# facebookresearch/actionmesh

Measured on AMD Instinct MI355X. Metric: denoise-steps/sec (16f x 4096tok), higher is better.
Workload: dtype bf16; 1 GPU; headline: Stage-I denoise step, B=2 (CFG) x T=16 frames x N=4096 tokens, width 1024 (8 heads x 128), 21 layers all inflated, S=257 ctx tokens, random-init weights, seeded N(0,1) latents/context resident in HBM; parallelism=single GPU

## Files before the change

actionmesh_amd/csrc/am_gemm.hip:

```cpp
#include <stdlib.h>
#include <string.h>

#include "am_common.h"

namespace {

constexpr int BM = 128, BN = 128, BK = 64;
constexpr int LDS_ROW = BK + 8;
constexpr int TILE_ELEMS = BM * LDS_ROW;
constexpr int CS_LD = BN + 4;
constexpr int SMEM_MAIN = 2 * 2 * TILE_ELEMS * (int)sizeof(bf16_t);
constexpr int SMEM_EPI = BM * CS_LD * (int)sizeof(float);
constexpr int SMEM_BYTES = SMEM_MAIN > SMEM_EPI ? SMEM_MAIN : SMEM_EPI;
constexpr int GROUP_M = 8;
constexpr int B2 = 256;

__device__ inline int64_t map_row(int r, int G, int gs, int off) {
  if (G <= 0) return r;
  int g = r / G;
  return (int64_t)g * gs + off + (r - g * G);
}

__global__ __launch_bounds__(256, 2) void gemm_bf16_kernel(am_gemm_args p, int tiles_m, int tiles_n, int m_base) {
  extern __shared__ __attribute__((aligned(16))) unsigned char smem[];
  bf16_t* As = reinterpret_cast<bf16_t*>(smem);
  bf16_t* Bs = As + 2 * TILE_ELEMS;
  float* Cs = reinterpret_cast<float*>(smem);

  const int nb = tiles_m * tiles_n;
  const int bid = blockIdx.x;
  int lid;
  {
    const int xcd = bid & 7, idx = bid >> 3;
    const int q = nb >> 3, r = nb & 7;
    lid = (xcd < r ? xcd * (q + 1) : r * (q + 1) + (xcd - r) * q) + idx;
  }
  int tm, tn;
  {
    const int group_sz = GROUP_M * tiles_n;
    const int g = lid / group_sz;
    const int first_m = g * GROUP_M;
    const int gm = min(GROUP_M, tiles_m - first_m);
    const int in_g = lid - g * group_sz;
    tm = first_m + in_g % gm;
    tn = in_g / gm;
  }
  const int m0 = m_base + tm * BM, n0 = tn * BN;

  const int tid = threadIdx.x;
  const int lane = tid & 63, wave = tid >> 6;
  const int l31 = lane & 31, hi = lane >> 5;
  const int wm = wave >> 1, wn = wave & 1;

  const bf16_t* a1p[4];
  const bf16_t* a2p[4];
  const bf16_t* wp[4];
  int lds_off[4];
#pragma unroll
  for (int i = 0; i < 4; ++i) {
    const int c = tid + 256 * i;
    const int row = c >> 3, col = (c & 7) * 8;
    const int ar = min(m0 + row, p.M - 1);
    const int64_t pr = map_row(ar, p.a_G, p.a_gs, p.a_off);
    a1p[i] = p.A1 + pr * p.lda1 + col;
    a2p[i] = p.A2 ? p.A2 + pr * p.lda2 + col - p.K1 : nullptr;
    const int wr = min(n0 + row, p.N - 1);
    wp[i] = p.W + (int64_t)wr * p.ldw + col;
    lds_off[i] = row * LDS_ROW + col;
  }

  f32x16_t acc[2][2];
#pragma unroll
  for (int i = 0; i < 2; ++i)
#pragma unroll
    for (int j = 0; j < 2; ++j)
#pragma unroll
      for (int r = 0; r < 16; ++r) acc[i][j][r] = 0.f;

  u32x4_t areg[4], wreg[4];
  auto load_tile = [&](int kt) {
    const int k0 = kt * BK;
    const bool first = k0 < p.K1;
#pragma unroll
    for (int i = 0; i < 4; ++i) {
      const bf16_t* src = first ? a1p[i] + k0 : a2p[i] + k0;
      areg[i] = *reinterpret_cast<const u32x4_t*>(src);
      wreg[i] = *reinterpret_cast<const u32x4_t*>(wp[i] + k0);
    }
  };
  auto store_tile = [&](int buf) {
#pragma unroll
    for (int i = 0; i < 4; ++i) {
      *reinterpret_cast<u32x4_t*>(&As[buf * TILE_ELEMS + lds_off[i]]) = areg[i];
      *reinterpret_cast<u32x4_t*>(&Bs[buf * TILE_ELEMS + lds_off[i]]) = wreg[i];
    }
  };

  const int nk = p.K / BK;
  load_tile(0);
  store_tile(0);

  const int a_frag_off = (wm * 64 + l31) * LDS_ROW + hi * 8;
  const int b_frag_off = (wn * 64 + l31) * LDS_ROW + hi * 8;

  for (int kt = 0; kt < nk; ++kt) {
    __syncthreads();
    const int buf = kt & 1;
    if (kt + 1 < nk) load_tile(kt + 1);
    const bf16_t* Ab = As + buf * TILE_ELEMS + a_frag_off;
    const bf16_t* Bb = Bs + buf * TILE_ELEMS + b_frag_off;
#pragma unroll
    for (int ks = 0; ks < BK / 16; ++ks) {
      bf16x8_t af[2], bfr[2];
#pragma unroll
      for (int i = 0; i < 2; ++i) {
        af[i] = *reinterpret_cast<const bf16x8_t*>(Ab + i * 32 * LDS_ROW + ks * 16);
        bfr[i] = *reinterpret_cast<const bf16x8_t*>(Bb + i * 32 * LDS_ROW + ks * 16);
      }
#pragma unroll
      for (int i = 0; i < 2; ++i)
#pragma unroll
        for (int j = 0; j < 2; ++j)
          acc[i][j] = AM_MFMA_32x32x16(bfr[j], af[i], acc[i][j]);
    }
    if (kt + 1 < nk) store_tile(buf ^ 1);
  }

  __syncthreads();
#pragma unroll
  for (int i = 0; i < 2; ++i)
#pragma unroll
    for (int j = 0; j < 2; ++j)
#pragma unroll
      for (int g = 0; g < 4; ++g) {
        const int m = wm * 64 + i * 32 + l31;
        const int n = wn * 64 + j * 32 + 8 * g + 4 * hi;
        f32x4_t v = {acc[i][j][4 * g], acc[i][j][4 * g + 1], acc[i][j][4 * g + 2], acc[i][j][4 * g + 3]};
        *reinterpret_cast<f32x4_t*>(&Cs[m * CS_LD + n]) = v;
      }
  __syncthreads();

  const int c8 = (tid & 15) * 8;
  const int gn = n0 + c8;
  if (gn < p.N) {
    float bv[8], cs[8];
#pragma unroll
    for (int e = 0; e < 8; ++e) {
      bv[e] = p.bias ? p.bias[gn + e] : 0.f;
      cs[e] = p.ln_stats ? p.ln_colsum[gn + e] : 0.f;
    }
#pragma unroll
    for (int pass = 0; pass < BM / 16; ++pass) {
      const int row = pass * 16 + (tid >> 4);
      const int gmr = m0 + row;
      if (gmr < p.M) {
        const int64_t pr = map_row(gmr, p.c_G, p.c_gs, p.c_off);
        const f32x4_t v0 = *reinterpret_cast<const f32x4_t*>(&Cs[row * CS_LD + c8]);
        const f32x4_t v1 = *reinterpret_cast<const f32x4_t*>(&Cs[row * CS_LD + c8 + 4]);
        float v[8] = {v0[0], v0[1], v0[2], v0[3], v1[0], v1[1], v1[2], v1[3]};
        if (p.ln_stats) {
          const f32x2_t st = *reinterpret_cast<const f32x2_t*>(p.ln_stats + 2 * map_row(gmr, p.a_G, p.a_gs, p.a_off));
          const float nm = -st[0] * st[1];
#pragma unroll
          for (int e = 0; e < 8; ++e) v[e] = rbf(fmaf(v[e], st[1], fmaf(nm, cs[e], bv[e])));
        } else {
#pragma unroll
          for (int e = 0; e < 8; ++e) v[e] = rbf(v[e] + bv[e]);
        }
        if ((p.act & AM_GEMM_ACT_MASK) == AM_GEMM_ACT_GELU) {
#pragma unroll
          for (int e = 0; e < 8; ++e) v[e] = rbf(gelu_erf(v[e]));
        }
        if (p.residual) {
          const u32x4_t rv = *reinterpret_cast<const u32x4_t*>(p.residual + pr * p.ldc + gn);
#pragma unroll
          for (int e = 0; e < 4; ++e) {
            v[2 * e] += bflo(rv[e]);
            v[2 * e + 1] += bfhi(rv[e]);
          }
        }
        u32x4_t o;
#pragma unroll
        for (int e = 0; e < 4; ++e) o[e] = pack_bf2(v[2 * e], v[2 * e + 1]);
        *reinterpret_cast<u32x4_t*>(p.C + pr * p.ldc + gn) = o;
      }
    }
  }
}


constexpr int TAIL_LD = 64 + 4;
__global__ __launch_bounds__(512) void gemm_tail_kernel(am_gemm_args p, int m_base) {
  __shared__ float red[4][32][TAIL_LD];
  const int tid = threadIdx.x;
  const int lane = tid & 63, wave = tid >> 6;
  const int l31 = lane & 31, hi = lane >> 5;
  const int wn = wave & 1, wk = wave >> 1;
  const int m0 = m_base + blockIdx.y * 32, nb0 = blockIdx.x * 64;
  const int ar = min(m0 + l31, p.M - 1);
  const int wr = min(nb0 + wn * 32 + l31, p.N - 1);
  const bf16_t* a1 = p.A1 + (int64_t)ar * p.lda1 + hi * 8;
  const bf16_t* a2 = p.A2 ? p.A2 + (int64_t)ar * p.lda2 + hi * 8 - p.K1 : nullptr;
  const bf16_t* wp = p.W + (int64_t)wr * p.ldw + hi * 8;
  const int kq = p.K >> 2;
  const int k_begin = wk * kq, k_end = k_begin + kq;
  f32x16_t acc;
#pragma unroll
  for (int r = 0; r < 16; ++r) acc[r] = 0.f;
  for (int k0 = k_begin; k0 < k_end; k0 += 128) {
    u32x4_t af[8], wf[8];
#pragma unroll
    for (int s = 0; s < 8; ++s) {
      const int k = min(k0 + s * 16, k_end - 16);
      af[s] = *reinterpret_cast<const u32x4_t*>((k < p.K1 ? a1 : a2) + k);
      wf[s] = *reinterpret_cast<const u32x4_t*>(wp + k);
    }
#pragma unroll
    for (int s = 0; s < 8; ++s)
      if (k0 + s * 16 < k_end)
        acc = AM_MFMA_32x32x16(__builtin_bit_cast(bf16x8_t, wf[s]), __builtin_bit_cast(bf16x8_t, af[s]), acc);
  }
#pragma unroll
  for (int g = 0; g < 4; ++g)
    *reinterpret_cast<f32x4_t*>(&red[wk][l31][wn * 32 + 8 * g + 4 * hi]) = f32x4_t{acc[4 * g], acc[4 * g + 1], acc[4 * g + 2], acc[4 * g + 3]};
  __syncthreads();
  const int row = tid >> 4, c4 = (tid & 15) * 4;
  const int gmr = m0 + row, gn = nb0 + c4;
  if (gmr >= p.M || gn >= p.N) return;
  float v[4];
  {
    const f32x4_t s0 = *reinterpret_cast<const f32x4_t*>(&red[0][row][c4]), s1 = *reinterpret_cast<const f32x4_t*>(&red[1][row][c4]);
    const f32x4_t s2 = *reinterpret_cast<const f32x4_t*>(&red[2][row][c4]), s3 = *reinterpret_cast<const f32x4_t*>(&red[3][row][c4]);
#pragma unroll
    for (int e = 0; e < 4; ++e) v[e] = (s0[e] + s1[e]) + (s2[e] + s3[e]);
  }
  float bv[4] = {0.f, 0.f, 0.f, 0.f};
  if (p.bias) {
    const f32x4_t b = *reinterpret_cast<const f32x4_t*>(p.bias + gn);
#pragma unroll
    for (int e = 0; e < 4; ++e) bv[e] = b[e];
  }
  if (p.ln_stats) {
    const f32x2_t st = *reinterpret_cast<const f32x2_t*>(p.ln_stats + 2 * (int64_t)gmr);
    const f32x4_t cs = *reinterpret_cast<const f32x4_t*>(p.ln_colsum + gn);
    const float nm = -st[0] * st[1];
#pragma unroll
    for (int e = 0; e < 4; ++e) v[e] = rbf(fmaf(v[e], st[1], fmaf(nm, cs[e], bv[e])));
  } else {
#pragma unroll
    for (int e = 0; e < 4; ++e) v[e] = rbf(v[e] + bv[e]);
  }
  if ((p.act & AM_GEMM_ACT_MASK) == AM_GEMM_ACT_GELU) {
#pragma unroll
    for (int e = 0; e < 4; ++e) v[e] = rbf(gelu_erf(v[e]));
  }
  if (p.residual) {
    const u32x2_t rv = *reinterpret_cast<const u32x2_t*>(p.residual + (int64_t)gmr * p.ldc + gn);
    v[0] += bflo(rv[0]); v[1] += bfhi(rv[0]); v[2] += bflo(rv[1]); v[3] += bfhi(rv[1]);
  }
  *reinterpret_cast<u32x2_t*>(p.C + (int64_t)gmr * p.ldc + gn) = u32x2_t{pack_bf2(v[0], v[1]), pack_bf2(v[2], v[3])};
}

#ifndef AM_GEMM_NT
#define AM_GEMM_NT 1
#endif
struct ResidualPrefetch {
  u32x4_t rv[16];
  bool on;
};
__device__ __forceinline__ bool residual_prefetchable(const am_gemm_args& p, int tid, int m0, int n0) {
  return p.residual != nullptr && p.c_G <= 0 && m0 + B2 <= p.M && n0 + (tid & 31) * 8 < p.N && !(p.act & AM_GEMM_ABLATE_MASK);
}
__device__ __forceinline__ void residual_prefetch(const am_gemm_args& p, int tid, int m0, int n0, ResidualPrefetch& r) {
  r.on = residual_prefetchable(p, tid, m0, n0);
  if (r.on) {
    const int k16 = tid & 31, r16 = tid >> 5;
    const uint32_t lane_off = ((uint32_t)r16 * (uint32_t)p.ldc + (uint32_t)(n0 + k16 * 8)) * 2u;
    const int64_t step = (int64_t)16 * p.ldc;
    const bf16_t* rrow = p.residual + (int64_t)m0 * p.ldc;
#pragma unroll
    for (int pass = 0; pass < 16; ++pass) {
      const u32x4_t* q = reinterpret_cast<const u32x4_t*>(reinterpret_cast<const unsigned char*>(rrow + pass * step) + lane_off);
      r.rv[pass] = AM_GEMM_NT ? __builtin_nontemporal_load(q) : *q;
    }
  }
}

__device__ __forceinline__ void emit_row_part(const u32x4_t& sv, float* part_row, bool writer) {
  float x[8];
#pragma unroll
  for (int e = 0; e < 4; ++e) { x[2 * e] = bflo(sv[e]); x[2 * e + 1] = bfhi(sv[e]); }
  float mean, m2;
  row_part8(x, mean, m2);
#define AM_CHAN_STEP(CTRL, ROWMASK, HALF_N)                                                                                  \
  {                                                                                                                          \
    const float om = __builtin_bit_cast(float, __builtin_amdgcn_update_dpp(__builtin_bit_cast(int, mean), __builtin_bit_cast(int, mean), CTRL, ROWMASK, 0xf, false)); \
    const float oq = __builtin_bit_cast(float, __builtin_amdgcn_update_dpp(__builtin_bit_cast(int, m2), __builtin_bit_cast(int, m2), CTRL, ROWMASK, 0xf, false));     \
    row_part_merge_equal(mean, m2, om, oq, HALF_N);                                                                          \
  }
  AM_CHAN_STEP(0xB1, 0xf, 4.f)
  AM_CHAN_STEP(0x4E, 0xf, 8.f)
  AM_CHAN_STEP(0x141, 0xf, 16.f)
  AM_CHAN_STEP(0x140, 0xf, 32.f)
  AM_CHAN_STEP(0x142, 0xa, 64.f)
#undef AM_CHAN_STEP
  if (writer) *reinterpret_cast<f32x2_t*>(part_row) = f32x2_t{mean, m2};
// ... 112 lines not shown
        u32x4_t u = *reinterpret_cast<const u32x4_t*>(su + pass * 8192);
        if (odd) u = u32x4_t{u[2], u[3], u[0], u[1]};
        float v[8];
#pragma unroll
        for (int e = 0; e < 4; ++e) {
          v[2 * e] = bflo(u[e]);
          v[2 * e + 1] = bfhi(u[e]);
        }
        if (wt) {
          float ss = 0.f;
#pragma unroll
          for (int e = 0; e < 8; ++e) ss = __builtin_fmaf(v[e], v[e], ss);
          ss += __builtin_bit_cast(float, __builtin_amdgcn_update_dpp(0, __builtin_bit_cast(int, ss), 0x128, 0xf, 0xf, false));
          ss += __builtin_bit_cast(float, __builtin_amdgcn_update_dpp(0, __builtin_bit_cast(int, ss), 0x124, 0xf, 0xf, false));
          ss += __builtin_bit_cast(float, __builtin_amdgcn_update_dpp(0, __builtin_bit_cast(int, ss), 0x122, 0xf, 0xf, false));
          ss += __builtin_bit_cast(float, __builtin_amdgcn_update_dpp(0, __builtin_bit_cast(int, ss), 0x121, 0xf, 0xf, false));
          const float r = rsqrtf(ss * (1.0f / 128.0f) + hp.eps);
#pragma unroll
          for (int e = 0; e < 8; ++e) v[e] = (v[e] * r) * wv[e];
        }
        if (hp.rope_cos) {
          f32x4_t cs, sn;
          if (two) {
            const bool nx = gm >= fb;
#pragma unroll
            for (int e = 0; e < 4; ++e) { cs[e] = nx ? cs1[e] : cs0[e]; sn[e] = nx ? sn1[e] : sn0[e]; }
          } else {
            const int frame = gm / hp.rows_per_frame;
            cs = *reinterpret_cast<const f32x4_t*>(hp.rope_cos + (int64_t)frame * 64 + sub * 4);
            sn = *reinterpret_cast<const f32x4_t*>(hp.rope_sin + (int64_t)frame * 64 + sub * 4);
          }
#pragma unroll
          for (int e = 0; e < 4; ++e) rope_rotate(v[2 * e], v[2 * e + 1], cs[e], sn[e]);
        }
        u32x4_t w;
#pragma unroll
        for (int e = 0; e < 4; ++e) w[e] = pack_bf2(v[2 * e], v[2 * e + 1]);
        if (two) {
          *reinterpret_cast<u32x4_t*>((gm >= sb ? out1 : out0) + (int64_t)gm * 128) = w;
        } else {
          const int seq = gm / hp.seq_len, sq = gm - seq * hp.seq_len;
          *reinterpret_cast<u32x4_t*>(out + (((int64_t)seq * hp.heads + head) * s_pad + sq) * 128 + sub * 8) = w;
        }
      };
      if (two && m0 + B2 <= p.M && wt != nullptr) {
        const bool rope = hp.rope_cos != nullptr;
#pragma unroll 1
        for (int b4 = 0; b4 < 16; b4 += 4) {
          u32x4_t u[4];
#pragma unroll
          for (int i = 0; i < 4; ++i) u[i] = *reinterpret_cast<const u32x4_t*>(su + (b4 + i) * 8192);
          float v[4][8], ss[4];
#pragma unroll
          for (int i = 0; i < 4; ++i) {
            if (odd) u[i] = u32x4_t{u[i][2], u[i][3], u[i][0], u[i][1]};
#pragma unroll
            for (int e = 0; e < 4; ++e) { v[i][2 * e] = bflo(u[i][e]); v[i][2 * e + 1] = bfhi(u[i][e]); }
            ss[i] = 0.f;
#pragma unroll
            for (int e = 0; e < 8; ++e) ss[i] = __builtin_fmaf(v[i][e], v[i][e], ss[i]);
          }
#define AM_HP_DPP(CTRL)                                                                                                         \
          _Pragma("unroll") for (int i = 0; i < 4; ++i)                                                                         \
            ss[i] += __builtin_bit_cast(float, __builtin_amdgcn_update_dpp(0, __builtin_bit_cast(int, ss[i]), CTRL, 0xf, 0xf, false));
          AM_HP_DPP(0x128) AM_HP_DPP(0x124) AM_HP_DPP(0x122) AM_HP_DPP(0x121)
#undef AM_HP_DPP
#pragma unroll
          for (int i = 0; i < 4; ++i) {
            const int gm = m0 + (b4 + i) * 16 + r16;
            const float r = __builtin_amdgcn_rsqf(ss[i] * (1.0f / 128.0f) + hp.eps);
#pragma unroll
            for (int e = 0; e < 8; ++e) v[i][e] = (v[i][e] * r) * wv[e];
            if (rope) {
              const bool nx = gm >= fb;
#pragma unroll
              for (int e = 0; e < 4; ++e) rope_rotate(v[i][2 * e], v[i][2 * e + 1], nx ? cs1[e] : cs0[e], nx ? sn1[e] : sn0[e]);
            }
            u32x4_t w;
#pragma unroll
            for (int e = 0; e < 4; ++e) w[e] = pack_bf2(v[i][2 * e], v[i][2 * e + 1]);
            *reinterpret_cast<u32x4_t*>((gm >= sb ? out1 : out0) + (int64_t)gm * 128) = w;
          }
        }
      } else if (two) {
#pragma unroll 4
        for (int pass = 0; pass < 16; ++pass) one_row(pass);
      } else {
#pragma unroll 2
        for (int pass = 0; pass < 16; ++pass) one_row(pass);
      }
    }
  }
  if (abl_nov) return;
#pragma unroll
  for (int h2 = 0; h2 < 2; ++h2) {
    const int pi = (n0 >> 7) + h2;
    const int head = pi / hp.nparts, part = pi - head * hp.nparts;
    if (n0 + h2 * 128 >= p.N || hp.kinds[part] != 2) continue;
    const int lane = tid & 63, wave = tid >> 6;
#pragma unroll 2
    for (int it = 0; it < 8; ++it) {
      const int pc = (lane & 7) + 8 * (it & 3);
      const int d = ((lane >> 3) & 7) + 8 * (wave + 8 * (it >> 2));
      const int pos0 = pc * 8;
      const int g16 = m0 + (pos0 & ~15);
      if (g16 >= p.M) continue;
      const int n = h2 * 128 + d;
      uint32_t val[8];
#pragma unroll
      for (int j = 0; j < 8; ++j) {
        const int pos = pos0 + j;
        const int m = (pos & ~15) | perm16(pos & 15);
        val[j] = *reinterpret_cast<const uint16_t*>(stage + m * 512 + ((((n >> 2) ^ (m & 15))) << 3) + (n & 3) * 2);
      }
      const u32x4_t w = {val[0] | (val[1] << 16), val[2] | (val[3] << 16), val[4] | (val[5] << 16), val[6] | (val[7] << 16)};
      const int seq = g16 / hp.seq_len, s16 = g16 - seq * hp.seq_len;
      *reinterpret_cast<u32x4_t*>(hp.out_vt + (((int64_t)seq * hp.heads + head) * 128 + d) * hp.sk_pad + s16 + (pos0 & 15)) = w;
    }
  }
}

constexpr int T2_UNITS = B2 * (BK / 8);
constexpr int T2_BYTES = T2_UNITS * 16;
constexpr int SMEM2_BYTES = 4 * T2_BYTES;

typedef __attribute__((address_space(3))) void* lds_ptr_t;
typedef const __attribute__((address_space(1))) void* gbl_ptr_t;

__global__ __launch_bounds__(512, 2) void gemm256_bf16_kernel(am_gemm_args p, int tiles_m, int tiles_n, int m_base) {
  extern __shared__ __attribute__((aligned(16))) unsigned char smem[];

  const int nb = tiles_m * tiles_n;
  const int bid = blockIdx.x;
  int lid;
  {
    const int xcd = bid & 7, idx = bid >> 3;
    const int q = nb >> 3, r = nb & 7;
    lid = (xcd < r ? xcd * (q + 1) : r * (q + 1) + (xcd - r) * q) + idx;
  }
  int tm, tn;
  {
    const int group_sz = GROUP_M * tiles_n;
    const int g = lid / group_sz;
    const int first_m = g * GROUP_M;
    const int gm = min(GROUP_M, tiles_m - first_m);
    const int in_g = lid - g * group_sz;
    tm = first_m + in_g % gm;
    tn = in_g / gm;
  }
  const int m0 = m_base + tm * B2, n0 = tn * B2;

  const int tid = threadIdx.x;
  const int lane = tid & 63;
  const int wave = __builtin_amdgcn_readfirstlane(tid >> 6);
  const int l31 = lane & 31, hi = lane >> 5;
  const int wm = wave >> 2, wn = wave & 3;

  const bf16_t* a1p[4];
  const bf16_t* a2p[4];
  const bf16_t* wp[4];
#pragma unroll
  for (int j = 0; j < 4; ++j) {
    const int U = j * 512 + wave * 64 + lane;
    const int r = U >> 3, c = (U & 7) ^ ((r >> 1) & 7);
    const int ar = min(m0 + r, p.M - 1);
    const int64_t pr = map_row(ar, p.a_G, p.a_gs, p.a_off);
    a1p[j] = p.A1 + pr * p.lda1 + c * 8;
    a2p[j] = p.A2 ? p.A2 + pr * p.lda2 + c * 8 - p.K1 : nullptr;
    const int wr = min(n0 + r, p.N - 1);
    wp[j] = p.W + (int64_t)wr * p.ldw + c * 8;
  }
  auto dma_pair = [&](int kt, int buf, int j) __attribute__((always_inline)) {
    const int k0 = kt * BK;
    unsigned char* abase = smem + buf * 2 * T2_BYTES;
    unsigned char* bbase = abase + T2_BYTES;
    const bf16_t* src = k0 < p.K1 ? a1p[j] + k0 : a2p[j] + k0;
    __builtin_amdgcn_global_load_lds((gbl_ptr_t)src, (lds_ptr_t)(abase + (j * 512 + wave * 64) * 16), 16, 0, 0);
    __builtin_amdgcn_global_load_lds((gbl_ptr_t)(wp[j] + k0), (lds_ptr_t)(bbase + (j * 512 + wave * 64) * 16), 16, 0, 0);
  };
  auto dma_tile = [&](int kt, int buf) {
#pragma unroll
    for (int j = 0; j < 4; ++j) dma_pair(kt, buf, j);
  };

  f32x16_t acc[4][2];
#pragma unroll
  for (int j = 0; j < 2; ++j)
#pragma unroll
    for (int g = 0; g < 4; ++g) {
      f32x4_t bv = {0.f, 0.f, 0.f, 0.f};
      if (p.bias) bv = *reinterpret_cast<const f32x4_t*>(p.bias + min(n0 + wn * 64 + j * 32 + 8 * g + 4 * hi, p.N - 4));
#pragma unroll
      for (int i = 0; i < 4; ++i)
#pragma unroll
        for (int e = 0; e < 4; ++e) acc[i][j][4 * g + e] = bv[e];
    }

  int a_row_off[4], a_sw[4], b_row_off[2], b_sw[2];
#pragma unroll
  for (int i = 0; i < 4; ++i) {
    const int R = wm * 128 + i * 32 + l31;
    a_row_off[i] = R * 128;
    a_sw[i] = (R >> 1) & 7;
  }
#pragma unroll
  for (int j = 0; j < 2; ++j) {
    const int R = wn * 64 + j * 32 + l31;
    b_row_off[j] = R * 128;
    b_sw[j] = (R >> 1) & 7;
  }

  const int nk = p.K / BK;
  dma_tile(0, 0);
  dma_drain_barrier();
  for (int kt = 0; kt < nk; ++kt) {
    const int buf = kt & 1;
    const int kn = min(kt + 1, nk - 1);
    const unsigned char* At = smem + buf * 2 * T2_BYTES;
    const unsigned char* Bt = At + T2_BYTES;
#pragma unroll
    for (int ks = 0; ks < BK / 16; ++ks) {
      if (ks < 2) {
        dma_pair(kn, buf ^ 1, 2 * ks);
        dma_pair(kn, buf ^ 1, 2 * ks + 1);
      }
      __builtin_amdgcn_sched_barrier(0);
      const int c = ks * 2 + hi;
      bf16x8_t af[4], bfr[2];
#pragma unroll
      for (int j = 0; j < 2; ++j)
        bfr[j] = *reinterpret_cast<const bf16x8_t*>(Bt + b_row_off[j] + ((c ^ b_sw[j]) << 4));
#pragma unroll
      for (int i = 0; i < 4; ++i)
        af[i] = *reinterpret_cast<const bf16x8_t*>(At + a_row_off[i] + ((c ^ a_sw[i]) << 4));
#pragma unroll
      for (int i = 0; i < 4; ++i)
#pragma unroll
        for (int j = 0; j < 2; ++j)
          acc[i][j] = AM_MFMA_32x32x16(bfr[j], af[i], acc[i][j]);
    }
    dma_drain_barrier();
  }

  unsigned char* stage = smem;
#pragma unroll
  for (int j = 0; j < 2; ++j)
#pragma unroll
    for (int g = 0; g < 4; ++g) {
      const int nl = wn * 64 + j * 32 + 8 * g + 4 * hi;
#pragma unroll
      for (int i = 0; i < 4; ++i) {
        const int ml = wm * 128 + i * 32 + l31;
        u32x2_t w;
        if ((p.act & AM_GEMM_ACT_MASK) == AM_GEMM_ACT_GELU) {
          float v[4];
#pragma unroll
          for (int e = 0; e < 4; ++e) v[e] = gelu_erf(rbf(acc[i][j][4 * g + e]));
          w = u32x2_t{pack_bf2(v[0], v[1]), pack_bf2(v[2], v[3])};
        } else {
          w = u32x2_t{pack_bf2(acc[i][j][4 * g], acc[i][j][4 * g + 1]), pack_bf2(acc[i][j][4 * g + 2], acc[i][j][4 * g + 3])};
        }
        const int u = (nl >> 2) ^ (ml & 15);
        *reinterpret_cast<u32x2_t*>(stage + ml * 512 + u * 8) = w;
      }
    }
  __syncthreads();
  store_staged_tile(p, stage, tid, m0, n0);
}


constexpr uint32_t GT_LO = (127u - 17u) << 7, GT_HI = (127u + 3u) << 7, GT_SPAN = GT_HI - GT_LO;
constexpr int GT_ENTRIES = 2 * (int)GT_SPAN;
constexpr int GT_BYTES = GT_ENTRIES * 2;
__global__ void gelu_table_kernel(uint16_t* tab) {
  const int i = blockIdx.x * blockDim.x + threadIdx.x;
  if (i >= GT_ENTRIES) return;
  const uint32_t sgn = (uint32_t)i / GT_SPAN, rel = (uint32_t)i - sgn * GT_SPAN;
  const bf16_t b = (bf16_t)((sgn << 15) | (rel + GT_LO));
  tab[i] = (uint16_t)(pack_bf2(gelu_erf(bf2f(b)), 0.f) & 0xffffu);
}
__device__ __forceinline__ uint32_t gelu_table_pair(uint32_t pk, const unsigned char* tab, uint32_t& bad) {
  const uint32_t b0 = pk & 0xffffu, b1 = pk >> 16;
  const uint32_t r0 = (b0 & 0x7fffu) - GT_LO, r1 = (b1 & 0x7fffu) - GT_LO;
  bad |= (uint32_t)(r0 >= GT_SPAN) | (uint32_t)(r1 >= GT_SPAN);
  const uint32_t i0 = min(r0, GT_SPAN - 1) + (b0 >> 15) * GT_SPAN, i1 = min(r1, GT_SPAN - 1) + (b1 >> 15) * GT_SPAN;
  const uint32_t g0 = *reinterpret_cast<const uint16_t*>(tab + 2u * i0);
  const uint32_t g1 = *reinterpret_cast<const uint16_t*>(tab + 2u * i1);
  return g0 | (g1 << 16);
}
__device__ __forceinline__ bool gelu_table_has(float x) {
  const uint32_t b = pack_bf2(x, 0.f) & 0x7fffu;
  return b - GT_LO < GT_SPAN;
}

constexpr int HT_BYTES = 128 * BK * 2;
constexpr int PBUF_BYTES = 4 * HT_BYTES;
constexpr int FOLD_OFF = 2 * PBUF_BYTES;
constexpr int SMEM2PP_BYTES = FOLD_OFF + 4096;
constexpr int GT_OFF = SMEM2PP_BYTES;
constexpr int SMEM2PP_GELU_BYTES = GT_OFF + GT_BYTES;

#define PP_BARRIER() do { __builtin_amdgcn_sched_barrier(0); asm volatile("s_barrier" ::: "memory"); __builtin_amdgcn_sched_barrier(0); } while (0)
#define PP_LGKM0() asm volatile("s_waitcnt lgkmcnt(0)" ::: "memory")

template <bool HP>
__global__ __launch_bounds__(512, 2) void gemm256pp_bf16_kernel(am_gemm_args p, int tiles_m, int tiles_n, int m_base, am_headpost_args hp,
                                                                 const uint16_t* gelu_tab) {
  extern __shared__ __attribute__((aligned(16))) unsigned char smem[];

  const int nb = tiles_m * tiles_n;
  const int bid = blockIdx.x;
  {
    const int units = (p.act & AM_GEMM_SKEW_MASK) >> AM_GEMM_SKEW_SHIFT;
    if (units && units < 7 && bid < 256) {
      const unsigned long long t0 = wall_clock64();
      const unsigned long long wait = (unsigned long long)(bid & 7) * units * 150ull;
      while (wall_clock64() - t0 < wait) __builtin_amdgcn_s_sleep(4);
    }
  }
  int lid;
  {
    const int xcd = bid & 7, idx = bid >> 3;
    const int q = nb >> 3, r = nb & 7;
    lid = (xcd < r ? xcd * (q + 1) : r * (q + 1) + (xcd - r) * q) + idx;
  }
  int tm, tn;
  {
    const int group_sz = GROUP_M * tiles_n;
    const int g = lid / group_sz;
    const int first_m = g * GROUP_M;
    const int gm = min(GROUP_M, tiles_m - first_m);
    const int in_g = lid - g * group_sz;
    tm = first_m + in_g % gm;
    tn = in_g / gm;
  }
  const int m0 = m_base + tm * B2, n0 = tn * B2;

  const int tid = threadIdx.x;
  const int lane = tid & 63;
  const int wave = __builtin_amdgcn_readfirstlane(tid >> 6);
  const int wm = wave >> 2, wn = wave & 3;

  const int l15 = lane & 15, l4 = lane >> 4;
  f32x4_t acc[8][4];
  {
    f32x4_t bv[4];
#pragma unroll
    for (int ni = 0; ni < 4; ++ni) {
      bv[ni] = f32x4_t{0.f, 0.f, 0.f, 0.f};
      if (p.bias && !p.ln_stats) bv[ni] = *reinterpret_cast<const f32x4_t*>(p.bias + min(n0 + wn * 64 + ni * 16 + l4 * 4, p.N - 4));
    }
#pragma unroll
    for (int ni = 0; ni < 4; ++ni) asm volatile("" : "+v"(bv[ni]));
#pragma unroll
    for (int ni = 0; ni < 4; ++ni)
#pragma unroll
      for (int mi = 0; mi < 8; ++mi) acc[mi][ni] = bv[ni];
  }
  __builtin_amdgcn_sched_barrier(0);
  if (p.ln_stats) {
    {
      const int dw = wave * 64 + lane;
      const int row = min(m0 + (dw >> 1), p.M - 1);
      __builtin_amdgcn_global_load_lds((gbl_ptr_t)(p.ln_stats + 2 * (int64_t)row + (dw & 1)), (lds_ptr_t)(smem + FOLD_OFF + wave * 256), 4, 0, 0);
    }
    {
      const int idx = (wave & 3) * 64 + lane;
      const int n = min(n0 + idx, p.N - 1);
      const float* src = wave < 4 ? p.ln_colsum + n : (p.bias ? p.bias + n : p.ln_colsum + n);
      __builtin_amdgcn_global_load_lds((gbl_ptr_t)src, (lds_ptr_t)(smem + FOLD_OFF + 2048 + wave * 256), 4, 0, 0);
    }
  }

  if (gelu_tab != nullptr) {
#pragma unroll
    for (int i = 0; i < GT_BYTES / 4 / 512; ++i)
      __builtin_amdgcn_global_load_lds((gbl_ptr_t)(reinterpret_cast<const uint32_t*>(gelu_tab) + i * 512 + wave * 64 + lane),
                                       (lds_ptr_t)(smem + GT_OFF + (i * 512 + wave * 64) * 4), 4, 0, 0);
  }

  uint32_t offA1[4], offA2[4], offW[4];
#pragma unroll
  for (int i = 0; i < 4; ++i) {
    const int half = i >> 1, pc = i & 1;
    const int r = pc * 64 + wave * 8 + (lane >> 3);
    const int c = (lane & 7) ^ ((r >> 1) & 7);
    const int ar = min(m0 + half * 128 + r, p.M - 1);
    const int64_t pr = map_row(ar, p.a_G, p.a_gs, p.a_off);
    offA1[i] = (uint32_t)(pr * (p.lda1 >> 3) + c);
    offA2[i] = (uint32_t)(pr * (p.lda2 >> 3) + c);
    const int wr = min(n0 + half * 128 + r, p.N - 1);
    offW[i] = (uint32_t)((int64_t)wr * (p.ldw >> 3) + c);
  }
  auto stage_a = [&](int half, int kt, int buf_off) __attribute__((always_inline)) {
    const int k0 = kt * BK;
    const bool first = k0 < p.K1;
    const unsigned char* base = reinterpret_cast<const unsigned char*>(first ? p.A1 + k0 : p.A2 + (k0 - p.K1));
#pragma unroll
    for (int pc = 0; pc < 2; ++pc) {
      const uint32_t off = first ? offA1[half * 2 + pc] : offA2[half * 2 + pc];
      __builtin_amdgcn_global_load_lds((gbl_ptr_t)(base + ((uint64_t)off << 4)),
                                       (lds_ptr_t)(smem + buf_off + half * HT_BYTES + (pc * 512 + wave * 64) * 16), 16, 0, 0);
    }
  };
  auto stage_w = [&](int half, int kt, int buf_off) __attribute__((always_inline)) {
    const unsigned char* base = reinterpret_cast<const unsigned char*>(p.W + kt * BK);
#pragma unroll
    for (int pc = 0; pc < 2; ++pc)
      __builtin_amdgcn_global_load_lds((gbl_ptr_t)(base + ((uint64_t)offW[half * 2 + pc] << 4)),
                                       (lds_ptr_t)(smem + buf_off + (2 + half) * HT_BYTES + (pc * 512 + wave * 64) * 16), 16, 0, 0);
  };


  const int fo0 = l15 * 128 + (((0 + l4) ^ (l15 >> 1)) << 4);
  const int fo1 = l15 * 128 + (((4 + l4) ^ (l15 >> 1)) << 4);
  const int a_base = wm * HT_BYTES;
  const int w_base = (2 + (wn >> 1)) * HT_BYTES + (wn & 1) * 64 * 128;

  bf16x8_t af[4][2], wf[4][2];
  auto read_a = [&](int cur, int mh) __attribute__((always_inline)) {
#pragma unroll
    for (int i = 0; i < 4; ++i) {
      const unsigned char* q = smem + cur + a_base + (mh * 4 + i) * 2048;
      af[i][0] = *reinterpret_cast<const bf16x8_t*>(q + fo0);
      af[i][1] = *reinterpret_cast<const bf16x8_t*>(q + fo1);
    }
  };
  auto read_w = [&](int cur, int nh) __attribute__((always_inline)) {
#pragma unroll
    for (int j = 0; j < 2; ++j) {
      const unsigned char* q = smem + cur + w_base + (nh * 2 + j) * 2048;
      wf[nh * 2 + j][0] = *reinterpret_cast<const bf16x8_t*>(q + fo0);
      wf[nh * 2 + j][1] = *reinterpret_cast<const bf16x8_t*>(q + fo1);
    }
  };
#define PP_QUADRANT(MH, NH)                                                                                       \
  do {                                                                                                            \
    __builtin_amdgcn_s_setprio(1);                                                                                \
    _Pragma("unroll") for (int ks = 0; ks < 2; ++ks)                                                              \
      _Pragma("unroll") for (int i = 0; i < 4; ++i)                                                               \
        _Pragma("unroll") for (int j = 0; j < 2; ++j)                                                             \
          acc[(MH) * 4 + i][(NH) * 2 + j] = AM_MFMA_16x16x32(                                                     \
              wf[(NH) * 2 + j][ks], af[i][ks], acc[(MH) * 4 + i][(NH) * 2 + j]);                                  \
    __builtin_amdgcn_s_setprio(0);                                                                                \
  } while (0)

  const int nk = p.K / BK;
  stage_a(0, 0, 0); stage_a(1, 0, 0); stage_w(0, 0, 0); stage_w(1, 0, 0);
  {
    const int t1 = min(1, nk - 1);
    stage_w(0, t1, PBUF_BYTES); stage_w(1, t1, PBUF_BYTES);
  }
  asm volatile("s_waitcnt vmcnt(4)" ::: "memory");
  PP_BARRIER();
  if (wm == 1) PP_BARRIER();

  for (int t = 0; t < nk; ++t) {
    const int cur = (t & 1) * PBUF_BYTES, nxt = PBUF_BYTES - cur;
    const int ta = min(t + 1, nk - 1), tb = min(t + 2, nk - 1);
    read_a(cur, 0); read_w(cur, 0);
    stage_a(0, ta, nxt);
    PP_LGKM0(); PP_BARRIER();
    PP_QUADRANT(0, 0);
    PP_BARRIER();
    read_w(cur, 1);
    stage_a(1, ta, nxt);
    PP_LGKM0(); PP_BARRIER();
    PP_QUADRANT(0, 1);
    PP_BARRIER();
    read_a(cur, 1);
    stage_w(0, tb, cur);
    PP_LGKM0(); PP_BARRIER();
    PP_QUADRANT(1, 1);
    PP_BARRIER();
    stage_w(1, tb, cur);
    asm volatile("s_waitcnt vmcnt(4)" ::: "memory");
    PP_BARRIER();
    PP_QUADRANT(1, 0);
    PP_BARRIER();
  }
  if (wm == 0) PP_BARRIER();
  asm volatile("s_waitcnt vmcnt(0)" ::: "memory");
  PP_BARRIER();

  ResidualPrefetch pre;
  pre.on = false;
  if constexpr (!HP) residual_prefetch(p, tid, m0, n0, pre);
  if (p.ln_stats) {
    f32x4_t cs[4], dv[4];
    const float* fold = reinterpret_cast<const float*>(smem + FOLD_OFF);
#pragma unroll
    for (int ni = 0; ni < 4; ++ni) {
      const int nl = wn * 64 + ni * 16 + l4 * 4;
      cs[ni] = *reinterpret_cast<const f32x4_t*>(fold + 512 + nl);
      dv[ni] = p.bias ? *reinterpret_cast<const f32x4_t*>(fold + 768 + nl) : f32x4_t{0.f, 0.f, 0.f, 0.f};
    }
#pragma unroll
    for (int mi = 0; mi < 8; ++mi) {
      const f32x2_t st = *reinterpret_cast<const f32x2_t*>(fold + 2 * (wm * 128 + mi * 16 + l15));
      const float nm = -st[0] * st[1];
#pragma unroll
      for (int ni = 0; ni < 4; ++ni)
#pragma unroll
        for (int e = 0; e < 4; ++e) acc[mi][ni][e] = fmaf(acc[mi][ni][e], st[1], fmaf(nm, cs[ni][e], dv[ni][e]));
    }
  }
  unsigned char* stage = smem;
  uint32_t gelu_bad = 0;
  auto stage_pass = [&](auto&& convert) __attribute__((always_inline)) {
#pragma unroll
    for (int mi = 0; mi < 8; ++mi)
#pragma unroll
      for (int ni = 0; ni < 4; ++ni) {
        const int ml = wm * 128 + mi * 16 + l15;
        const int nl = wn * 64 + ni * 16 + l4 * 4;
        const u32x2_t w = convert(acc[mi][ni]);
        const int u = (nl >> 2) ^ (ml & 15);
        *reinterpret_cast<u32x2_t*>(stage + ml * 512 + u * 8) = w;
      }
  };
  if ((p.act & AM_GEMM_ACT_MASK) == AM_GEMM_ACT_GELU && gelu_tab != nullptr) {
    stage_pass([&](const f32x4_t& a) __attribute__((always_inline)) {
      return u32x2_t{gelu_table_pair(pack_bf2(a[0], a[1]), smem + GT_OFF, gelu_bad), gelu_table_pair(pack_bf2(a[2], a[3]), smem + GT_OFF, gelu_bad)};
    });
  } else if ((p.act & AM_GEMM_ACT_MASK) == AM_GEMM_ACT_GELU) {
    stage_pass([&](const f32x4_t& a) __attribute__((always_inline)) {
      float v[4];
#pragma unroll
      for (int e = 0; e < 4; ++e) v[e] = gelu_erf(rbf(a[e]));
      return u32x2_t{pack_bf2(v[0], v[1]), pack_bf2(v[2], v[3])};
    });
  } else {
    stage_pass([&](const f32x4_t& a) __attribute__((always_inline)) { return u32x2_t{pack_bf2(a[0], a[1]), pack_bf2(a[2], a[3])}; });
  }
  if (gelu_bad) {
#pragma unroll
    for (int mi = 0; mi < 8; ++mi)
#pragma unroll
      for (int ni = 0; ni < 4; ++ni) {
        const int ml = wm * 128 + mi * 16 + l15;
        const int nl = wn * 64 + ni * 16 + l4 * 4;
        bool any = false;
#pragma unroll
        for (int e = 0; e < 4; ++e) any |= !gelu_table_has(acc[mi][ni][e]);
        if (any) {
          uint16_t* q = reinterpret_cast<uint16_t*>(stage + ml * 512 + ((nl >> 2) ^ (ml & 15)) * 8);
#pragma unroll
          for (int e = 0; e < 4; ++e)
            if (!gelu_table_has(acc[mi][ni][e])) q[e] = (uint16_t)(pack_bf2(gelu_erf(rbf(acc[mi][ni][e])), 0.f) & 0xffffu);
        }
      }
  }
  __syncthreads();
  if constexpr (HP) store_staged_tile_headpost(p, hp, stage, tid, m0, n0);
  else store_staged_tile(p, stage, tid, m0, n0, &pre);
}
#undef PP_QUADRANT

}

static int gemm_skew_units(int rounds) {
  static int enabled[64];
  int dev = 0;
  if (hipGetDevice(&dev) != hipSuccess || dev < 0 || dev >= 64) return 0;
  if (enabled[dev] == 0) {
    hipDeviceProp_t pr;
    bool on = hipGetDeviceProperties(&pr, dev) == hipSuccess && pr.multiProcessorCount == 256 && strncmp(pr.gcnArchName, "gfx950", 6) == 0;
    const char* e = getenv("ACTIONMESH_AMD_GEMM_SKEW");
    if (e && e[0] == '0') on = false;
    enabled[dev] = on ? 1 : 2;
  }
  if (enabled[dev] != 1) return 0;
  return rounds >= 24 ? 4 : rounds >= 16 ? 3 : rounds >= 12 ? 2 : rounds >= 4 ? 1 : 0;
}

static const uint16_t* gelu_table(hipStream_t st) {
#ifdef AM_F16
  return nullptr;
#else
  static uint16_t* tab[64];
  static int state[64];
  static std::mutex mu;
  int dev = 0, cur = 0;
  if (hipGetDevice(&cur) != hipSuccess) return nullptr;
  dev = cur;
  if (st != nullptr && hipStreamGetDevice(st, &dev) != hipSuccess) { (void)hipGetLastError(); dev = cur; }
  if (dev < 0 || dev >= 64) return nullptr;
  std::lock_guard<std::mutex> lk(mu);
  if (state[dev] == 0) {
    const char* e = getenv("ACTIONMESH_AMD_GELU_TABLE");
    if (e && e[0] == '0') { state[dev] = 2; return nullptr; }
    hipStreamCaptureStatus cs = hipStreamCaptureStatusNone;
    if (hipStreamIsCapturing(st, &cs) != hipSuccess || cs != hipStreamCaptureStatusNone) { (void)hipGetLastError(); return nullptr; }
    if (dev != cur && hipSetDevice(dev) != hipSuccess) { (void)hipGetLastError(); return nullptr; }
    uint16_t* t = nullptr;
    bool ok = hipMalloc(reinterpret_cast<void**>(&t), GT_BYTES) == hipSuccess;
    if (ok) {
      hipLaunchKernelGGL(gelu_table_kernel, dim3(ceil_div(GT_ENTRIES, 256)), dim3(256), 0, st, t);
      ok = hipGetLastError() == hipSuccess && hipStreamSynchronize(st) == hipSuccess;
      if (!ok) (void)hipFree(t);
    }
    if (dev != cur) (void)hipSetDevice(cur);
    if (!ok) { (void)hipGetLastError(); return nullptr; }
    tab[dev] = t;
    state[dev] = 1;
  }
  return state[dev] == 1 ? tab[dev] : nullptr;
#endif
}

int am_row_part(const bf16_t* Cmat, int ldc, int64_t row0, int64_t rows, int N, float* part, void* stream);

static void launch_tail(const am_gemm_args& args, int m_main, hipStream_t st) {
  static int use128 = -1;
  if (use128 < 0) { const char* e = getenv("ACTIONMESH_AMD_GEMM_TAIL"); use128 = (e && strcmp(e, "128") == 0) ? 1 : 0; }
  const int rows = args.M - m_main;
  if (!use128 && args.a_G == 0 && args.c_G == 0 && rows <= 128 && args.N % 4 == 0 && ((uintptr_t)args.bias % 16 == 0)) {
    hipLaunchKernelGGL(gemm_tail_kernel, dim3(ceil_div(args.N, 64), ceil_div(rows, 32)), dim3(512), 0, st, args, m_main);
  } else {
    const int tn = ceil_div(args.N, BN);
    hipLaunchKernelGGL(gemm_bf16_kernel, dim3(tn), dim3(256), SMEM_BYTES, st, args, 1, tn, m_main);
  }
}

struct Gemm256Plan {
  bool big;
  int rem, m_main, tiles_m, tiles_n;
  int skew;
};
static Gemm256Plan gemm256_plan(int M, int N, int act, bool skew_counts_tail) {
  Gemm256Plan p;
  p.big = !(act & AM_GEMM_FORCE_128) && N >= 8 && M >= 1 &&
          ((act & AM_GEMM_FORCE_256) || (N >= 256 && M >= 1024 && (int64_t)ceil_div(M, B2) * ceil_div(N, B2) >= 192));
  p.rem = M % B2;
  p.m_main = (p.rem != 0 && p.rem <= 128 && M > 8 * B2) ? M - p.rem : M;
  p.tiles_m = ceil_div(p.m_main, B2), p.tiles_n = ceil_div(N, B2);
  p.skew = act & AM_GEMM_SKEW_MASK;
  if (p.big && p.skew == 0)
    p.skew = gemm_skew_units((int)(((int64_t)(skew_counts_tail ? ceil_div(M, B2) : p.tiles_m) * p.tiles_n) / 256)) << AM_GEMM_SKEW_SHIFT;
  return p;
}
static int gemm_set_lds_attributes() {
  const std::pair<const void*, int> kernels[] = {{(const void*)gemm_bf16_kernel, SMEM_BYTES}, {(const void*)gemm256_bf16_kernel, SMEM2_BYTES},
      {(const void*)gemm256pp_bf16_kernel<false>, SMEM2PP_GELU_BYTES}, {(const void*)gemm256pp_bf16_kernel<true>, SMEM2PP_BYTES}};
  AM_ONCE_PER_DEVICE({ for (const auto& k : kernels) AM_HIP(hipFuncSetAttribute(k.first, hipFuncAttributeMaxDynamicSharedMemorySize, k.second)); });
  return AM_OK;
}

extern "C" int am_gemm_bf16(const am_gemm_args* a, void* stream) {
  AM_CHECK(a != nullptr, "am_gemm_bf16: null args");
  AM_CHECK(a->M > 0 && a->N > 0 && a->K > 0, "am_gemm_bf16: empty problem M=%d N=%d K=%d", a->M, a->N, a->K);
  AM_CHECK(a->K % BK == 0, "am_gemm_bf16: K=%d must be a multiple of %d", a->K, BK);
  AM_CHECK(a->N % 8 == 0, "am_gemm_bf16: N=%d must be a multiple of 8", a->N);
  AM_CHECK(a->A1 && a->W && a->C, "am_gemm_bf16: null operand");
  AM_CHECK(a->K1 > 0 && a->K1 <= a->K && a->K1 % BK == 0, "am_gemm_bf16: K1=%d invalid for K=%d", a->K1, a->K);
  AM_CHECK(a->K1 == a->K || a->A2 != nullptr, "am_gemm_bf16: K1 < K requires A2");
  AM_CHECK(a->lda1 % 8 == 0 && a->ldw % 8 == 0 && a->ldc % 8 == 0 && (a->A2 == nullptr || a->lda2 % 8 == 0),
           "am_gemm_bf16: leading dimensions must be multiples of 8 elements (16 B)");
  AM_CHECK(((uintptr_t)a->A1 | (uintptr_t)a->W | (uintptr_t)a->C | (uintptr_t)a->A2 | (uintptr_t)a->residual) % 16 == 0,
           "am_gemm_bf16: operands must be 16-byte aligned");
  if (a->ln_stats) {
    AM_CHECK(a->ln_colsum != nullptr, "am_gemm_bf16: ln_stats without ln_colsum");
    AM_CHECK(a->A2 == nullptr, "am_gemm_bf16: a folded LayerNorm needs one A operand");
    AM_CHECK(a->a_G == 0 || (a->act & AM_GEMM_FORCE_128) || (a->N < 256 && !(a->act & AM_GEMM_FORCE_256)),
             "am_gemm_bf16: a folded LayerNorm over a row-mapped A needs the 128x128 kernel (N < 256 without the forced 256x256 tile)");
    AM_CHECK(!(a->act & AM_GEMM_LOCKSTEP), "am_gemm_bf16: the round-1 lockstep kernel has no folded-LayerNorm epilogue");
    AM_CHECK(((uintptr_t)a->ln_stats % 8 == 0) && ((uintptr_t)a->ln_colsum % 16 == 0) && (a->bias == nullptr || (uintptr_t)a->bias % 16 == 0) &&
             a->N % 4 == 0, "am_gemm_bf16: ln_stats / ln_colsum / bias misaligned");
  }
  if (a->ln_part) {
    AM_CHECK(a->c_G == 0, "am_gemm_bf16: ln_part needs the identity C row map");
    AM_CHECK((uintptr_t)a->ln_part % 8 == 0, "am_gemm_bf16: ln_part misaligned");
  }
  AM_TRY(gemm_set_lds_attributes());
  am_gemm_args args = *a;
  const bool legacy = (args.act & AM_GEMM_LOCKSTEP) != 0;
  const int abl = args.act & AM_GEMM_ABLATE_MASK;
  const bool no_gelu_table = (args.act & AM_GEMM_NO_GELU_TABLE) != 0;
  args.act &= AM_GEMM_ACT_MASK;
  AM_CHECK(args.act == 0 || args.act == AM_GEMM_ACT_GELU, "am_gemm_bf16: unknown activation %d", args.act);
  const Gemm256Plan plan = gemm256_plan(args.M, args.N, a->act, true);
  AM_CHECK(!plan.big || (uintptr_t)args.bias % 16 == 0, "am_gemm_bf16: the 256x256 tile needs a 16-byte aligned bias");
  args.act |= abl | plan.skew;
  float* const ln_part = args.ln_part;
  int64_t part_done = 0;
  args.ln_part = nullptr;
  if (plan.big) {
    const int m_main = plan.m_main, tiles_m = plan.tiles_m, tiles_n = plan.tiles_n;
    if (legacy) {
      hipLaunchKernelGGL(gemm256_bf16_kernel, dim3(tiles_m * tiles_n), dim3(512), SMEM2_BYTES,
                         (hipStream_t)stream, args, tiles_m, tiles_n, 0);
    } else {
      am_gemm_args main_args = args;
      if (ln_part && args.N % B2 == 0 && !(args.act & AM_GEMM_ABLATE_MASK)) {
        main_args.ln_part = ln_part;
        part_done = (int64_t)(args.M / B2) * B2;
        if (part_done > m_main) part_done = m_main;
      }
      const uint16_t* gt = ((main_args.act & AM_GEMM_ACT_MASK) == AM_GEMM_ACT_GELU && !no_gelu_table) ? gelu_table((hipStream_t)stream) : nullptr;
      hipLaunchKernelGGL(gemm256pp_bf16_kernel<false>, dim3(tiles_m * tiles_n), dim3(512), gt ? SMEM2PP_GELU_BYTES : SMEM2PP_BYTES,
                         (hipStream_t)stream, main_args, tiles_m, tiles_n, 0, am_headpost_args{}, gt);
    }
    if (m_main < args.M) launch_tail(args, m_main, (hipStream_t)stream);
  } else {
    const int tiles_m = ceil_div(args.M, BM), tiles_n = ceil_div(args.N, BN);
    hipLaunchKernelGGL(gemm_bf16_kernel, dim3(tiles_m * tiles_n), dim3(256), SMEM_BYTES,
                       (hipStream_t)stream, args, tiles_m, tiles_n, 0);
  }
  AM_HIP(hipGetLastError());
  if (ln_part && part_done < args.M)
    AM_TRY(am_row_part(args.C, args.ldc, part_done, args.M - part_done, args.N, ln_part, stream));
  return AM_OK;
}

int am_head_post_partial(const am_headpost_args* a, int s_min_last, int s_min_other, void* stream);

extern "C" int am_gemm_headpost_bf16(const am_gemm_args* g, const am_headpost_args* hp, void* stream) {
  AM_CHECK(g && hp, "am_gemm_headpost_bf16: null argument");
  AM_CHECK(g->C == hp->X && g->ldc == hp->ldx && (int64_t)g->M == hp->rows && g->N == hp->heads * hp->nparts * 128,
           "am_gemm_headpost_bf16: the GEMM's output (C, ldc, M, N) must be the head split's input (X, ldx, rows, heads * nparts * 128)");
  bool has_v = false;
  for (int i = 0; i < hp->nparts; ++i) has_v |= hp->kinds[i] == 2;
  const Gemm256Plan plan = gemm256_plan(g->M, g->N, g->act & AM_GEMM_ABLATE_MASK, false);
  AM_CHECK(g->ln_part == nullptr, "am_gemm_headpost_bf16: no row statistics of a head-split output");
  const bool fuse = (g->act & AM_GEMM_ACT_MASK) == 0 && !g->residual && (!g->bias || g->ln_stats) && !g->A2 && g->a_G == 0 && g->c_G == 0 && g->N % 256 == 0 && g->M % 16 == 0 &&
                    plan.big && (!has_v || hp->seq_len % 16 == 0) && (plan.m_main == g->M || plan.rem <= hp->seq_len) && hp->rows % hp->seq_len == 0 &&
                    !(g->act & (AM_GEMM_FORCE_128 | AM_GEMM_LOCKSTEP | AM_GEMM_FORCE_256)) && getenv("ACTIONMESH_AMD_NO_FUSED_QKV") == nullptr;
  if (!fuse) {
    AM_TRY(am_gemm_bf16(g, stream));
    return am_head_post(hp, stream);
  }
  AM_CHECK(g->K % BK == 0 && g->K1 == g->K && g->lda1 % 8 == 0 && g->ldw % 8 == 0, "am_gemm_headpost_bf16: bad GEMM operands");
  AM_CHECK(((uintptr_t)g->A1 | (uintptr_t)g->W | (uintptr_t)g->C) % 16 == 0, "am_gemm_headpost_bf16: operands must be 16-byte aligned");
  if (g->ln_stats)
    AM_CHECK(g->ln_colsum && (uintptr_t)g->ln_stats % 8 == 0 && (uintptr_t)g->ln_colsum % 16 == 0 && (g->bias == nullptr || (uintptr_t)g->bias % 16 == 0),
             "am_gemm_headpost_bf16: ln_stats / ln_colsum / bias missing or misaligned");
  AM_TRY(am_head_post_check(hp));
  AM_TRY(gemm_set_lds_attributes());
  am_gemm_args args = *g;
  args.act = (g->act & AM_GEMM_ABLATE_MASK) | plan.skew;
  const int m_main = plan.m_main, tiles_m = plan.tiles_m, tiles_n = plan.tiles_n;
  am_gemm_args main_args = args;
  main_args.M = m_main;
  hipLaunchKernelGGL(gemm256pp_bf16_kernel<true>, dim3(tiles_m * tiles_n), dim3(512), SMEM2PP_BYTES, (hipStream_t)stream, main_args, tiles_m,
                     tiles_n, 0, *hp, (const uint16_t*)nullptr);
  if (m_main < args.M) launch_tail(args, m_main, (hipStream_t)stream);
  AM_HIP(hipGetLastError());
  const int s_min_last = hp->seq_len - (args.M - m_main);
  return am_head_post_partial(hp, s_min_last, hp->seq_len, stream);
}
```

Before: 1.589 denoise-steps/s.

## Re-schedule gemm256pp LDS-DMA prefetch with compile-time verified stage table

Moves the global-to-LDS staging schedule of the ping-pong GEMM into a constexpr table. A tiles are now prefetched two k-tiles ahead and W tiles one ahead, reversing the previous order. Staging is split into per-piece loads spread across quadrant intervals, with tuned vmcnt waits. A constexpr replay simulator checks at compile time that there are no buffer hazards for small nk. The aim is to hide more of the load latency behind MFMA work, at the cost of more in-flight loads and a more complex schedule.

New measurement: 1.595 denoise-steps/s (median of 6 runs). No clear change (+0.4%).

```diff
diff --git a/actionmesh_amd/csrc/am_gemm.hip b/actionmesh_amd/csrc/am_gemm.hip
--- a/actionmesh_amd/csrc/am_gemm.hip
+++ b/actionmesh_amd/csrc/am_gemm.hip
@@ -2,6 +2,7 @@
 #include <string.h>
 
 #include "am_common.h"
+#include "am_gemm_schedule.h"
 
 namespace {
 
@@ -720,6 +721,7 @@
 
 #define PP_BARRIER() do { __builtin_amdgcn_sched_barrier(0); asm volatile("s_barrier" ::: "memory"); __builtin_amdgcn_sched_barrier(0); } while (0)
 #define PP_LGKM0() asm volatile("s_waitcnt lgkmcnt(0)" ::: "memory")
+#define PP_VMCNT(N) asm volatile("s_waitcnt vmcnt(%0)" ::"n"(N) : "memory")
 
 template <bool HP>
 __global__ __launch_bounds__(512, 2) void gemm256pp_bf16_kernel(am_gemm_args p, int tiles_m, int tiles_n, int m_base, am_headpost_args hp,
@@ -810,23 +812,31 @@
     const int wr = min(n0 + half * 128 + r, p.N - 1);
     offW[i] = (uint32_t)((int64_t)wr * (p.ldw >> 3) + c);
   }
-  auto stage_a = [&](int half, int kt, int buf_off) __attribute__((always_inline)) {
-    const int k0 = kt * BK;
-    const bool first = k0 < p.K1;
-    const unsigned char* base = reinterpret_cast<const unsigned char*>(first ? p.A1 + k0 : p.A2 + (k0 - p.K1));
-#pragma unroll
-    for (int pc = 0; pc < 2; ++pc) {
-      const uint32_t off = first ? offA1[half * 2 + pc] : offA2[half * 2 + pc];
-      __builtin_amdgcn_global_load_lds((gbl_ptr_t)(base + ((uint64_t)off << 4)),
-                                       (lds_ptr_t)(smem + buf_off + half * HT_BYTES + (pc * 512 + wave * 64) * 16), 16, 0, 0);
+  const int nk = p.K / BK;
+  auto stage_piece = [&](int op, int pc, int kt, int buf_off) __attribute__((always_inline)) {
+    const int k0 = min(kt, nk - 1) * BK;
+    if (op == pp_sched::OP_A) {
+      const bool first = k0 < p.K1;
+      const unsigned char* base = reinterpret_cast<const unsigned char*>(first ? p.A1 + k0 : p.A2 + (k0 - p.K1));
+#pragma unroll
+      for (int half = 0; half < 2; ++half) {
+        const uint32_t off = first ? offA1[half * 2 + pc] : offA2[half * 2 + pc];
+        __builtin_amdgcn_global_load_lds((gbl_ptr_t)(base + ((uint64_t)off << 4)),
+                                         (lds_ptr_t)(smem + buf_off + half * HT_BYTES + (pc * 512 + wave * 64) * 16), 16, 0, 0);
+      }
+    } else {
+      const unsigned char* base = reinterpret_cast<const unsigned char*>(p.W + k0);
+#pragma unroll
+      for (int half = 0; half < 2; ++half)
+        __builtin_amdgcn_global_load_lds((gbl_ptr_t)(base + ((uint64_t)offW[half * 2 + pc] << 4)),
+                                         (lds_ptr_t)(smem + buf_off + (2 + half) * HT_BYTES + (pc * 512 + wave * 64) * 16), 16, 0, 0);
     }
   };
-  auto stage_w = [&](int half, int kt, int buf_off) __attribute__((always_inline)) {
-    const unsigned char* base = reinterpret_cast<const unsigned char*>(p.W + kt * BK);
-#pragma unroll
-    for (int pc = 0; pc < 2; ++pc)
-      __builtin_amdgcn_global_load_lds((gbl_ptr_t)(base + ((uint64_t)offW[half * 2 + pc] << 4)),
-                                       (lds_ptr_t)(smem + buf_off + (2 + half) * HT_BYTES + (pc * 512 + wave * 64) * 16), 16, 0, 0);
+  auto stage_interval = [&](int at, int t, int cur) __attribute__((always_inline)) {
+#pragma unroll
+    for (int e = 0; e < pp_sched::NSTAGES; ++e)
+      if (pp_sched::STAGES[e].at == at)
+        stage_piece(pp_sched::STAGES[e].op, pp_sched::STAGES[e].pc, t + pp_sched::STAGES[e].dist, pp_sched::STAGES[e].other ? PBUF_BYTES - cur : cur);
   };
 
 
@@ -863,36 +873,33 @@
     __builtin_amdgcn_s_setprio(0);                                                                                \
   } while (0)
 
-  const int nk = p.K / BK;
-  stage_a(0, 0, 0); stage_a(1, 0, 0); stage_w(0, 0, 0); stage_w(1, 0, 0);
-  {
-    const int t1 = min(1, nk - 1);
-    stage_w(0, t1, PBUF_BYTES); stage_w(1, t1, PBUF_BYTES);
-  }
-  asm volatile("s_waitcnt vmcnt(4)" ::: "memory");
+#pragma unroll
+  for (int e = 0; e < pp_sched::NFIRST; ++e)
+    stage_piece(pp_sched::PROLOGUE[e].op, pp_sched::PROLOGUE[e].pc, pp_sched::PROLOGUE[e].tile, (pp_sched::PROLOGUE[e].tile & 1) * PBUF_BYTES);
+  PP_VMCNT(pp_sched::PROLOGUE_KEEP);
   PP_BARRIER();
   if (wm == 1) PP_BARRIER();
 
   for (int t = 0; t < nk; ++t) {
-    const int cur = (t & 1) * PBUF_BYTES, nxt = PBUF_BYTES - cur;
-    const int ta = min(t + 1, nk - 1), tb = min(t + 2, nk - 1);
+    const int cur = (t & 1) * PBUF_BYTES;
     read_a(cur, 0); read_w(cur, 0);
-    stage_a(0, ta, nxt);
+    stage_interval(pp_sched::R1, t, cur);
     PP_LGKM0(); PP_BARRIER();
     PP_QUADRANT(0, 0);
     PP_BARRIER();
     read_w(cur, 1);
-    stage_a(1, ta, nxt);
+    stage_interval(pp_sched::R2, t, cur);
+    PP_VMCNT(pp_sched::WAITS[0].keep);
     PP_LGKM0(); PP_BARRIER();
     PP_QUADRANT(0, 1);
     PP_BARRIER();
     read_a(cur, 1);
-    stage_w(0, tb, cur);
+    stage_interval(pp_sched::R3, t, cur);
     PP_LGKM0(); PP_BARRIER();
     PP_QUADRANT(1, 1);
     PP_BARRIER();
-    stage_w(1, tb, cur);
-    asm volatile("s_waitcnt vmcnt(4)" ::: "memory");
+    stage_interval(pp_sched::R4, t, cur);
+    PP_VMCNT(pp_sched::WAITS[1].keep);
     PP_BARRIER();
     PP_QUADRANT(1, 0);
     PP_BARRIER();
diff --git a/actionmesh_amd/csrc/am_gemm_schedule.h b/actionmesh_amd/csrc/am_gemm_schedule.h
--- /dev/null
+++ b/actionmesh_amd/csrc/am_gemm_schedule.h
@@ -0,0 +1,100 @@
+#pragma once
+
+namespace pp_sched {
+
+enum { R1 = 0, R2 = 1, R3 = 2, R4 = 3 };
+enum { OP_A = 0, OP_W = 1 };
+
+struct Stage { int op, pc, dist, other, at; };
+struct Read  { int op, pc, at; };
+struct Wait  { int at, keep; };
+struct First { int op, pc, tile; };
+
+constexpr Stage STAGES[] = {
+    {OP_W, 0, 1, 1, R1}, {OP_W, 1, 1, 1, R1},
+    {OP_A, 0, 2, 0, R2},
+    {OP_A, 1, 2, 0, R4},
+};
+constexpr Read READS[] = {
+    {OP_A, 0, R1}, {OP_W, 0, R1}, {OP_W, 1, R1},
+    {OP_W, 0, R2}, {OP_W, 1, R2},
+    {OP_A, 1, R3},
+};
+constexpr Wait WAITS[] = {{R2, 10}, {R4, 4}};
+constexpr First PROLOGUE[] = {
+    {OP_A, 0, 0}, {OP_W, 0, 0}, {OP_W, 1, 0}, {OP_A, 1, 0}, {OP_A, 0, 1}, {OP_A, 1, 1},
+};
+constexpr int PROLOGUE_KEEP = 6;
+constexpr int INSTR_PER_ENTRY = 2;
+constexpr int LOOP_KEEP = WAITS[1].keep;
+constexpr int LOOP_IN_FLIGHT = 12;
+
+template <class T, int N> constexpr int count_of(const T (&)[N]) { return N; }
+constexpr int NSTAGES = count_of(STAGES), NREADS = count_of(READS), NWAITS = count_of(WAITS), NFIRST = count_of(PROLOGUE);
+
+constexpr int replay(int nk) {
+  constexpr int NEVER = 1 << 30;
+  int gen[8] = {}, owed[8] = {}, last_read[8] = {}, ready[8][2] = {};
+  for (int c = 0; c < 8; ++c) { gen[c] = -NEVER; owed[c] = 0; last_read[c] = -NEVER; ready[c][0] = ready[c][1] = NEVER; }
+  int q_piece[2][64] = {}, q_gen[2][64] = {}, head[2] = {0, 0}, tail[2] = {0, 0};
+
+  auto reads_of = [](int op, int pc) { int n = 0; for (int r = 0; r < NREADS; ++r) n += (READS[r].op == op && READS[r].pc == pc) ? 2 : 0; return n; };
+  int err = 0;
+  auto issue = [&](int g, int slot, int buf, int op, int pc, int tile) {
+    const int c = buf * 4 + op * 2 + pc;
+    if (gen[c] != tile) {
+      if (owed[c] != 0 || last_read[c] >= slot) err = err ? err : 1;
+      gen[c] = tile;
+      owed[c] = (tile >= 0 && tile < nk) ? reads_of(op, pc) : 0;
+      ready[c][0] = ready[c][1] = NEVER;
+    }
+    q_piece[g][tail[g]] = c; q_gen[g][tail[g]] = tile; ++tail[g];
+  };
+  auto wait = [&](int g, int slot, int keep) {
+    while ((tail[g] - head[g]) * INSTR_PER_ENTRY > keep) {
+      const int c = q_piece[g][head[g]];
+      if (gen[c] == q_gen[g][head[g]]) ready[c][g] = slot;
+      ++head[g];
+    }
+  };
+
+  for (int g = 0; g < 2; ++g) {
+    for (int e = 0; e < NFIRST; ++e) issue(g, -1, PROLOGUE[e].tile & 1, PROLOGUE[e].op, PROLOGUE[e].pc, PROLOGUE[e].tile);
+    wait(g, -1, PROLOGUE_KEEP);
+  }
+  for (int slot = 0; slot < 8 * nk + 1; ++slot) {
+    const int g = slot & 1, s0 = slot - g;
+    if ((s0 & 1) || s0 >= 8 * nk) continue;
+    const int t = s0 >> 3, at = (s0 & 7) >> 1, buf = t & 1;
+    for (int e = 0; e < NSTAGES; ++e)
+      if (STAGES[e].at == at) issue(g, slot, STAGES[e].other ? buf ^ 1 : buf, STAGES[e].op, STAGES[e].pc, t + STAGES[e].dist);
+    for (int r = 0; r < NREADS; ++r)
+      if (READS[r].at == at) {
+        const int c = buf * 4 + READS[r].op * 2 + READS[r].pc;
+        if (gen[c] != t) err = err ? err : 2;
+        else if (ready[c][0] >= slot || ready[c][1] >= slot) err = err ? err : 3;
+        last_read[c] = slot;
+        owed[c] -= 1;
+      }
+    for (int w = 0; w < NWAITS; ++w)
+      if (WAITS[w].at == at) {
+        const int in_flight = (tail[g] - head[g]) * INSTR_PER_ENTRY;
+        if (in_flight < WAITS[w].keep) err = err ? err : 5;
+        if (w == NWAITS - 1 && in_flight != LOOP_IN_FLIGHT) err = err ? err : 4;
+        wait(g, slot, WAITS[w].keep);
+        if (w == NWAITS - 1) {
+          if ((tail[g] - head[g]) * INSTR_PER_ENTRY != LOOP_KEEP) err = err ? err : 4;
+          for (int i = head[g]; i < tail[g]; ++i)
+            if (q_gen[g][i] != t + 2 || ((q_piece[g][i] >> 1) & 1) != OP_A) err = err ? err : 4;
+        }
+      }
+  }
+  for (int c = 0; c < 8; ++c)
+    if (owed[c] != 0) err = err ? err : 2;
+  return err;
+}
+
+static_assert(replay(1) == 0 && replay(2) == 0 && replay(3) == 0 && replay(4) == 0, "gemm256pp LDS-DMA schedule: nk = 1 ... 4");
+static_assert(replay(5) == 0 && replay(6) == 0 && replay(7) == 0 && replay(8) == 0, "gemm256pp LDS-DMA schedule: nk = 5 ... 8");
+
+}
```
